# ArseneAmoya/image-retrieval-wavelet

Hardware: AMD Instinct MI355X
Metric: query images/sec + mAP@5000, MIRFLICKR-25k 64-bit hash, 1/2/4/8 MI355X (higher is better)
Workload: dtype f32; 1 GPU; c1: MIRFLICKR-25k shape, retrieval-only: per GPU per step 2048 query images 3x224x224 u8 -> SWT db2 L3 -> band-attention head (Nq=4, E=384; DINOv2 backbone out of scope, CLS features synthetic) -> 64-bit hash -> Hamming top-5000 vs 25,000 codes -> mAP@5000; queries_per_gpu=2048, db_codes=25000, nbits=64, k=5000, wavelet=db2, level=3, arithmetic=fp32 SWT and head (fp32 MFMA), 64-bit popcount ranking, AP in fp32/fp64, streams=1, clock_steps=40, backend=none, parallelism=single GPU

## Files before the change

### image-retrieval-wavelet_amd/csrc/ap_walk.hpp

```cpp
#pragma once
#include "common.hpp"

namespace wv {

constexpr int kApRounds = 32;

template <int TPQ>
__host__ __device__ constexpr int ap_scratch_dwords() { return kApRounds * (TPQ / 64) + 2 * (TPQ / 64) + 2; }

struct ApState {
    uint32_t running = 0;
    double acc = 0.0;
};

template <int TPQ>
__device__ __forceinline__ void ap_accum(uint32_t relbits, const uint32_t *cnt, int Rc, int r_base, int t, ApState &st)
{
    constexpr int NW = TPQ / 64, CH = 8;
    const int wv = t >> 6;
    for (int r0 = 0; r0 < Rc; r0 += CH) {
        uint32_t c[CH][NW];
#pragma unroll
        for (int u = 0; u < CH; ++u)
#pragma unroll
            for (int w2 = 0; w2 < NW; ++w2) c[u][w2] = cnt[min(r0 + u, Rc - 1) * NW + w2];
#pragma unroll
        for (int u = 0; u < CH; ++u) {
            const int r = r0 + u;
            if (r < Rc) {
                uint32_t before = st.running, tot = 0;
#pragma unroll
                for (int w2 = 0; w2 < NW; ++w2) {
                    before += w2 < wv ? c[u][w2] : 0u;
                    tot += c[u][w2];
                }
                const bool rel = (relbits >> r) & 1u;
                const uint64_t m = __ballot(rel);
                if (rel) {
                    const uint32_t j = before + (uint32_t)mbcnt(m) + 1;
                    st.acc += (double)((float)j / (float)((r_base + r) * TPQ + t + 1));
                }
                st.running += tot;
            }
        }
    }
}

template <int TPQ, typename SYNC>
__device__ __forceinline__ void ap_final(const ApState &st, double *wsum, int t, float *__restrict__ ap_out,
                                         int32_t *__restrict__ nrel_out, SYNC group_barrier)
{
    constexpr int NW = TPQ / 64;
    const int lane = t & 63, wv = t >> 6;
    const double acc = wave_sum_f64(st.acc);
    if (lane == 0) wsum[wv] = acc;
    group_barrier();
    if (t == 0) {
        double s = wsum[0];
#pragma unroll
        for (int w2 = 1; w2 < NW; ++w2) s += wsum[w2];
        *ap_out = st.running ? (float)(s / (double)st.running) : 0.0f;
        if (nrel_out) *nrel_out = (int32_t)st.running;
    }
}

constexpr int kMaxCutoffs = 16;

struct ApCuts {
    int n;
    int k[kMaxCutoffs];
};

template <int TPQ>
__host__ __device__ constexpr int ap_cuts_scratch_dwords() { return ap_scratch_dwords<TPQ>() + TPQ / 64; }

template <int TPQ, typename SYNC>
__device__ __forceinline__ void ap_accum_cuts(uint32_t relbits, const uint32_t *cnt, int Rc, int r_base, int t, ApState &st,
                                              const ApCuts &cuts, int &next, double *wsum, uint32_t *wcut,
                                              float *__restrict__ ap_out, int32_t *__restrict__ nrel_out, SYNC group_barrier)
{
    constexpr int NW = TPQ / 64, CH = 8;
    const int lane = t & 63, wv = t >> 6;
    int64_t cut = next < cuts.n ? cuts.k[next] : INT64_MAX;
    for (int r0 = 0; r0 < Rc; r0 += CH) {
        uint32_t c[CH][NW];
#pragma unroll
        for (int u = 0; u < CH; ++u)
#pragma unroll
            for (int w2 = 0; w2 < NW; ++w2) c[u][w2] = cnt[min(r0 + u, Rc - 1) * NW + w2];
#pragma unroll
        for (int u = 0; u < CH; ++u) {
            const int r = r0 + u;
            if (r < Rc) {
                uint32_t before = st.running, tot = 0;
#pragma unroll
                for (int w2 = 0; w2 < NW; ++w2) {
                    before += w2 < wv ? c[u][w2] : 0u;
                    tot += c[u][w2];
                }
                const bool rel = (relbits >> r) & 1u;
                const uint64_t m = __ballot(rel);
                const int p = (r_base + r) * TPQ + t;
                double own = 0.0;
                if (rel) {
                    const uint32_t j = before + (uint32_t)mbcnt(m) + 1;
                    own = (double)((float)j / (float)(p + 1));
                }
                while (cut <= (int64_t)(r_base + r + 1) * TPQ) {
                    const bool in = rel && p < cut;
                    const uint64_t mc = __ballot(in);
                    const double acc = wave_sum_f64(in ? st.acc + own : st.acc);
                    if (lane == 0) {
                        wsum[wv] = acc;
                        wcut[wv] = (uint32_t)__popcll(mc);
                    }
                    group_barrier();
                    if (t == 0) {
                        double s = wsum[0];
                        uint32_t running = st.running + wcut[0];
#pragma unroll
                        for (int w2 = 1; w2 < NW; ++w2) {
                            s += wsum[w2];
                            running += wcut[w2];
                        }
                        ap_out[next] = running ? (float)(s / (double)running) : 0.0f;
                        if (nrel_out) nrel_out[next] = (int32_t)running;
                    }
                    group_barrier();
                    ++next;
                    cut = next < cuts.n ? cuts.k[next] : INT64_MAX;
                }
                if (rel) st.acc += own;
                st.running += tot;
            }
        }
    }
}

}
```

### image-retrieval-wavelet_amd/csrc/rank.hpp

```cpp
#pragma once
#include "common.hpp"

namespace wv {

struct ApCuts;

constexpr int kTopkThreads = 256;
constexpr int kMaxBins = 130;
constexpr int kWinBins = 32;
constexpr int kWinRows = kWinBins + 1;
constexpr size_t kRankLdsLimit = 100 * 1024;

enum class RankKernel {
    none,
    column,
    window256,
    window64,
};

enum class RankMode {
    lists,
    rows16,
    hist,
    ap,
    relbits,
    radius,
};

constexpr int64_t kImg64MaxRows = 64 * 64;
constexpr int64_t kImg256MaxRows = 256 * 128;

constexpr int rank_threads_per_query(RankKernel kern) { return kern == RankKernel::window64 ? 64 : 256; }

struct RankPlan {
    RankKernel kernel;
    int C;
    int NC;
    size_t lds;
    const char *why;
    const char *instead;
};

__host__ __device__ inline int rank2_bitmap_words(int64_t N) { return (int)((N + 31) / 32); }

inline size_t window_lds_bytes_per_query(int tpq, int k, int bm_words = 0)
{
    size_t b = (size_t)kWinRows * (tpq / 2) * 4;
    b += ((size_t)(k + tpq) * 2 + 15) / 16 * 16;
    b += (size_t)(kMaxBins + 1 + kWinBins + 4 + 3) / 4 * 4 * 4;
    b += (size_t)bm_words * 4;
    b = (b + 15) / 16 * 16;
    const size_t hist = (size_t)(kMaxBins + 1) * 17 * 4;
    return b > hist ? b : (hist + 15) / 16 * 16;
}

constexpr int rank_radius_bitmap_words(int C) { return 8 * C + 1; }
inline size_t radius_lds_bytes(int C)
{
    const size_t b = (size_t)(kMaxBins + 1) * 16 * 4 + (size_t)2 * (kMaxBins + 1) * 4 + (size_t)rank_radius_bitmap_words(C) * 4;
    return (b + 15) / 16 * 16;
}

inline bool column_u16(int64_t n_items) { return n_items < 65536; }
inline size_t column_lds_bytes(int nbins, bool u16)
{
    const size_t h = (size_t)nbins * (u16 ? kTopkThreads / 2 : kTopkThreads);
    return (h + kMaxBins + kMaxBins + 1 + 4 + 3) / 4 * 4 * sizeof(uint32_t);
}

inline RankPlan rank_plan_column(int64_t N, int nbits)
{
    return {RankKernel::column, (int)ceil_div(N, kTopkThreads), 0, column_lds_bytes(nbits + 1, column_u16(N)), nullptr, ""};
}

inline RankKernel rank_window_kernel(int Q, int64_t N, int k)
{
    const char *force = ::wv::tune("WV_TOPK_V2");
    if (force && force[0] == '0') return RankKernel::none;
    if (N >= 65536 || 2 * (k + 128) >= 65536) return RankKernel::none;
    const bool fits256 = N <= kImg256MaxRows && window_lds_bytes_per_query(256, k) <= kRankLdsLimit;
    const bool fits64 = N <= kImg64MaxRows && 4 * window_lds_bytes_per_query(64, k) <= kRankLdsLimit;
    if (force && atoi(force) == 64 && fits64) return RankKernel::window64;
    if (force && atoi(force) == 256 && fits256) return RankKernel::window256;
    if (fits64 && Q >= 4096) return RankKernel::window64;
    return fits256 ? RankKernel::window256 : (fits64 ? RankKernel::window64 : RankKernel::none);
}

inline RankPlan rank_plan(int Q, int64_t N, int nbits, int k, RankMode mode)
{
    const bool fused = mode == RankMode::ap || mode == RankMode::relbits;
    const char *instead = mode == RankMode::ap ? "; call wv_hamming_topk + wv_map_at_k instead" : "";
    RankKernel kern = rank_window_kernel(Q, N, std::max(k, 1));
    if (kern == RankKernel::none) {
        if (mode == RankMode::lists) return rank_plan_column(N, nbits);
        return {RankKernel::none, 0, 0, 0, "are outside the windowed kernel (rows <= 32768, 16-bit row numbers: 2 (k + 128) < 65536)",
                instead};
    }
    if (fused && kern == RankKernel::window64 && k > 32 * 64) kern = RankKernel::window256;
    if (mode == RankMode::radius) kern = RankKernel::window256;
    RankPlan p{kern, 0, 0, 0, nullptr, ""};
    const int tpq = rank_threads_per_query(kern);
    p.C = (int)ceil_div(N, tpq);
    p.NC = p.C <= 16 ? 4 : (p.C <= 32 ? 8 : (p.C <= 64 ? 16 : (p.C <= 100 ? 25 : 32)));
    p.lds = window_lds_bytes_per_query(tpq, k, fused ? rank2_bitmap_words(N) : 0) * (kTopkThreads / tpq);
    if (mode == RankMode::radius) p.lds = radius_lds_bytes(p.C);
    if (fused && p.lds > kRankLdsLimit)
        return {RankKernel::none, 0, 0, 0, "do not fit the fused kernel's LDS (list + relevance bitmap)", instead};
    return p;
}

inline int rank_refuse(const char *what, const RankPlan &p, int64_t N, int k)
{
    WV_FAIL(WV_ENOTSUP, "%s: %lld rows / k=%d %s%s", what, (long long)N, k, p.why, p.instead);
}

inline size_t rank_image_bytes(RankKernel kern, int64_t N, int words)
{
    if (kern == RankKernel::column) return (size_t)ceil_div(N, kTopkThreads) * kTopkThreads * words * sizeof(uint64_t);
    const int tpq = rank_threads_per_query(kern);
    const int64_t C = ceil_div(N, tpq), rows = words == 1 ? (C + 1) / 2 : C;
    return (size_t)rows * tpq * 16;
}

struct BlobLayout {
    size_t column, window256, window64, total;
};
inline BlobLayout blob_layout(int64_t N, int words)
{
    BlobLayout L;
    L.column = L.window256 = L.window64 = L.total = (size_t)align_up((int64_t)dist_prepared_bytes(N, words), 256);
    if (words > 2) return L;
    L.window256 = L.column + (size_t)align_up((int64_t)rank_image_bytes(RankKernel::column, N, words), 256);
    L.window64 = L.window256 + (N <= kImg256MaxRows ? (size_t)align_up((int64_t)rank_image_bytes(RankKernel::window256, N, words), 256) : 0);
    L.total = L.window64 + (N <= kImg64MaxRows ? rank_image_bytes(RankKernel::window64, N, words) : 0);
    return L;
}
inline const void *blob_image(const void *prepared, int64_t N, int words, RankKernel kern)
{
    const BlobLayout L = blob_layout(N, words);
    return (const char *)prepared + (kern == RankKernel::column ? L.column : (kern == RankKernel::window256 ? L.window256 : L.window64));
}

int rank2_prepare(const uint64_t *db, void *img, int64_t N, int words, RankKernel kern, hipStream_t st);
size_t rank2_labels_bytes(int64_t N, int lwords);
int rank2_labels_prepare(const uint64_t *dblab, void *cls, int64_t N, int lwords, hipStream_t st);

struct Rank2Ap {
    const uint32_t *cls;
    const uint64_t *qlab;
    int lwords;
    float *ap;
    int32_t *nrel;
    uint64_t *relbits;
    int64_t relbits_ld;
    int64_t cum_ld;
};

int rank2_launch(const RankPlan &plan, const uint64_t *q, const void *img, int32_t *idx, uint16_t *rows16, uint8_t *dist,
                 uint32_t *cum, int Q, int64_t N, int nbits, int k, int64_t idx_offset, hipStream_t st,
                 const Rank2Ap *apx = nullptr, const ApCuts *cuts = nullptr);

int rank2_radius_launch(const RankPlan &plan, const uint64_t *q, const void *img, const Rank2Ap &apx, uint32_t *cum, uint32_t *cumrel,
                        int Q, int64_t N, int nbits, hipStream_t st);

}
```

### image-retrieval-wavelet_amd/csrc/rank2.hip

```cpp
#include "rank.hpp"
#include "ap_walk.hpp"

namespace wv {

#ifdef WV_RANK2_STAMPS
__device__ unsigned long long g_rank2_stamps[8];
#define R2_STAMP(i) do { __builtin_amdgcn_sched_barrier(0); const unsigned long long now_ = __builtin_amdgcn_s_memtime(); \
    __builtin_amdgcn_s_waitcnt(0xC07F); if (t == 0) atomicAdd(&g_rank2_stamps[i], now_ - stamp_); stamp_ = __builtin_amdgcn_s_memtime(); \
    __builtin_amdgcn_sched_barrier(0); } while (0)
#define R2_STAMP_INIT unsigned long long stamp_ = __builtin_amdgcn_s_memtime()
#else
#define R2_STAMP(i) do { } while (0)
#define R2_STAMP_INIT do { } while (0)
#endif

template <int WORDS>
struct QCode {
    uint64_t w[WORDS];
};

template <int TPQ>
__device__ __forceinline__ void group_sync()
{
    if constexpr (TPQ == 64) {
        __builtin_amdgcn_fence(__ATOMIC_ACQ_REL, "wavefront");
        __builtin_amdgcn_wave_barrier();
    } else {
        __syncthreads();
    }
}

__device__ __forceinline__ uint32_t wave_min_u32(uint32_t v)
{
#pragma unroll
    for (int d = 32; d > 0; d >>= 1) v = min(v, (uint32_t)__shfl_xor((int)v, d, 64));
    return v;
}

struct Rank2Lds {
    uint32_t *table;
    uint16_t *stage;
    uint32_t *gbase;
    uint32_t *tot;
    uint32_t *misc;
};

template <int WORDS, int TPQ, int NC>
__device__ __forceinline__ void rank2_distances(const uint4 *__restrict__ img, const QCode<WORDS> &qc, int64_t N, int C,
                                                int t, uint32_t (&dc)[NC], uint32_t &dmin)
{
    constexpr int UNR = WORDS == 1 ? 16 : 8;
    constexpr int LPB = WORDS == 1 ? UNR / 2 : UNR;
    const int first = t * C;
    const int nvalid = min(C, max(0, (int)N - first));
    const int rows = WORDS == 1 ? (C + 1) / 2 : C;
    const uint32_t toff = (uint32_t)t * 16u;
    dmin = 255;
#pragma unroll
    for (int i = 0; i < NC; ++i) dc[i] = 0xffffffffu;
#pragma unroll
    for (int bi = 0; bi < (NC * 4 + UNR - 1) / UNR; ++bi) {
        if (bi * UNR < C) {
            uint4 raw[LPB];
#pragma unroll
            for (int u = 0; u < LPB; ++u)
                raw[u] = *reinterpret_cast<const uint4 *>(reinterpret_cast<const char *>(img) +
                                                          (size_t)min(bi * LPB + u, rows - 1) * (TPQ * 16) + toff);
#pragma unroll
            for (int u4 = 0; u4 < UNR / 4; ++u4) {
                if (bi * (UNR / 4) + u4 >= NC) continue;
                uint32_t word = 0;
#pragma unroll
                for (int j = 0; j < 4; ++j) {
                    const int u = 4 * u4 + j;
                    uint32_t d;
                    if constexpr (WORDS == 1) {
                        const uint4 v = raw[u >> 1];
                        const uint32_t lo32 = (u & 1) ? v.z : v.x, hi32 = (u & 1) ? v.w : v.y;
                        d = (uint32_t)__popc(lo32 ^ (uint32_t)qc.w[0]) + (uint32_t)__popc(hi32 ^ (uint32_t)(qc.w[0] >> 32));
                    } else {
                        const uint4 v = raw[u];
                        d = (uint32_t)__popc(v.x ^ (uint32_t)qc.w[0]) + (uint32_t)__popc(v.y ^ (uint32_t)(qc.w[0] >> 32)) +
                            (uint32_t)__popc(v.z ^ (uint32_t)qc.w[1]) + (uint32_t)__popc(v.w ^ (uint32_t)(qc.w[1] >> 32));
                    }
                    dmin = min(dmin, d);
                    word |= d << (8 * j);
                }
                dc[bi * (UNR / 4) + u4] = word;
            }
        }
    }
#pragma unroll
    for (int i = 0; i < NC; ++i) {
        const int keep = min(4, max(0, C - 4 * i));
        dc[i] |= keep >= 4 ? 0u : (0xffffffffu << (8 * keep));
    }
    if (nvalid < C) {
#pragma unroll
        for (int i = 0; i < NC; ++i) {
            const int keep = min(4, max(0, nvalid - 4 * i));
            dc[i] |= keep >= 4 ? 0u : (0xffffffffu << (8 * keep));
        }
    }
}

template <int TPQ, int NC>
__device__ __forceinline__ void rank2_hist_only(const uint32_t (&dc)[NC], int64_t N, int C, int nbins,
                                                uint32_t *__restrict__ cum_out, uint8_t *lds_raw, int t)
{
    uint32_t *table = reinterpret_cast<uint32_t *>(lds_raw);
    uint32_t *tot = table + (kMaxBins + 1) * 16;
    for (int i = t; i < (nbins + 1) * 16; i += TPQ) table[i] = 0;
    group_sync<TPQ>();
    const uint32_t c = (uint32_t)(t & 31);
    const uint32_t cell_addr = (c >> 1) * 4u, cell_inc = 1u << (16 * (c & 1));
    char *tbl = reinterpret_cast<char *>(table);
#pragma unroll
    for (int bw = 0; bw < NC; bw += 2) {
        if (bw * 4 < C) {
#pragma unroll
            for (int j = 0; j < 8; ++j) {
                if (bw + (j >> 2) < NC) {
                    const uint32_t d = (dc[bw + (j >> 2)] >> (8 * (j & 3))) & 0xffu;
                    const uint32_t b = min(d, (uint32_t)nbins);
                    __hip_atomic_fetch_add(reinterpret_cast<uint32_t *>(tbl + b * 64 + cell_addr), cell_inc,
                                           __ATOMIC_RELAXED, __HIP_MEMORY_SCOPE_WORKGROUP);
                }
            }
            __builtin_amdgcn_sched_barrier(0);
        }
    }
    group_sync<TPQ>();
    for (int b = t; b < nbins; b += TPQ) {
        const uint4 *row = reinterpret_cast<const uint4 *>(table + b * 16);
        uint32_t s = 0;
#pragma unroll
        for (int i = 0; i < 4; ++i) {
            const uint4 v = row[i];
            s += (v.x & 0xffffu) + (v.x >> 16) + (v.y & 0xffffu) + (v.y >> 16) + (v.z & 0xffffu) + (v.z >> 16) +
                 (v.w & 0xffffu) + (v.w >> 16);
        }
        tot[b] = s;
    }
    group_sync<TPQ>();
    if (t < 64) {
        const int b0 = 3 * t;
        const uint32_t t0 = b0 < nbins ? tot[b0] : 0u, t1 = b0 + 1 < nbins ? tot[b0 + 1] : 0u, t2 = b0 + 2 < nbins ? tot[b0 + 2] : 0u;
        const uint32_t incl = wave_incl_scan_u32(t0 + t1 + t2), excl = incl - (t0 + t1 + t2);
        if (b0 <= nbins) cum_out[b0] = excl;
        if (b0 + 1 <= nbins) cum_out[b0 + 1] = excl + t0;
        if (b0 + 2 <= nbins) cum_out[b0 + 2] = excl + t0 + t1;
    }
    group_sync<TPQ>();
    (void)N;
}

template <int TPQ>
__device__ __forceinline__ void rank2_relevance_bitmap(const uint32_t *__restrict__ cls, uint64_t ql, uint64_t ql_hi, int nw, int t,
                                                       uint32_t *bitmap)
{
    constexpr int WPT = 4;
    uint32_t acc[WPT] = {0u, 0u, 0u, 0u};
    int wi[WPT];
#pragma unroll
    for (int i = 0; i < WPT; ++i) wi[i] = min(t + i * TPQ, nw - 1);
    uint64_t m = ql;
    int cbase = 0;
    if (!m) { m = ql_hi; ql_hi = 0; cbase = 64; }
    while (m) {
        const int c0 = cbase + __builtin_ctzll(m);
        m &= m - 1;
        const int c1 = m ? cbase + __builtin_ctzll(m) : c0;
        m &= m - 1;
        const int c2 = m ? cbase + __builtin_ctzll(m) : c0;
        m &= m - 1;
        const int c3 = m ? cbase + __builtin_ctzll(m) : c0;
        m &= m - 1;
        uint32_t v[4][WPT];
#pragma unroll
        for (int i = 0; i < WPT; ++i) {
            v[0][i] = cls[(size_t)c0 * nw + wi[i]];
            v[1][i] = cls[(size_t)c1 * nw + wi[i]];
            v[2][i] = cls[(size_t)c2 * nw + wi[i]];
            v[3][i] = cls[(size_t)c3 * nw + wi[i]];
        }
#pragma unroll
        for (int i = 0; i < WPT; ++i) acc[i] |= (v[0][i] | v[1][i]) | (v[2][i] | v[3][i]);
        if (!m && ql_hi) { m = ql_hi; ql_hi = 0; cbase = 64; }
    }
#pragma unroll
    for (int i = 0; i < WPT; ++i)
        if (t + i * TPQ < nw) bitmap[t + i * TPQ] = acc[i];
    for (int w = t + WPT * TPQ; w < nw; w += TPQ) bitmap[w] = 0;
}

template <int TPQ>
__device__ __forceinline__ void rank2_ap(const uint16_t *stage, const uint32_t *bitmap, uint32_t *scratch, int k, int t,
                                         float *__restrict__ ap_out, int32_t *__restrict__ nrel_out,
                                         uint64_t *__restrict__ relbits_out)
{
    constexpr int NW = TPQ / 64;
    const int lane = t & 63, wv = t >> 6;
    const int R = (k + TPQ - 1) / TPQ;
    uint32_t *cnt = scratch;
    double *wsum = reinterpret_cast<double *>(scratch + kApRounds * NW + (kApRounds * NW & 1));
    constexpr int CH = 8;
    ApState st;
    for (int c0 = 0; c0 < R; c0 += kApRounds) {
        const int Rc = min(kApRounds, R - c0);
        uint32_t relbits = 0;
        for (int r0 = c0; r0 < c0 + Rc; r0 += CH) {
            uint32_t it[CH], wd[CH];
#pragma unroll
            for (int u = 0; u < CH; ++u) it[u] = stage[min((r0 + u) * TPQ + t, k - 1)];
#pragma unroll
            for (int u = 0; u < CH; ++u) wd[u] = bitmap[it[u] >> 5];
#pragma unroll
            for (int u = 0; u < CH; ++u) {
                const int r = r0 + u;
                const bool rel = r < c0 + Rc && r * TPQ + t < k && ((wd[u] >> (it[u] & 31)) & 1u);
                relbits |= (rel ? 1u : 0u) << ((r - c0) & 31);
                const uint64_t m = __ballot(rel);
                if (lane == 0 && r < c0 + Rc) {
                    if (!relbits_out) cnt[(r - c0) * NW + wv] = (uint32_t)__popcll(m);
                    else if ((r * NW + wv) * 64 < k) relbits_out[r * NW + wv] = m;
                }
            }
        }
        if (relbits_out) continue;
        group_sync<TPQ>();
        ap_accum<TPQ>(relbits, cnt, Rc, c0, t, st);
        group_sync<TPQ>();
    }
    if (relbits_out) return;
    ap_final<TPQ>(st, wsum, t, ap_out, nrel_out, [] { group_sync<TPQ>(); });
}
template <int TPQ>
__device__ __forceinline__ void rank2_ap_cuts(const uint16_t *stage, const uint32_t *bitmap, uint32_t *scratch, int k, int t,
                                              float *__restrict__ ap_out, int32_t *__restrict__ nrel_out, const ApCuts &cuts)
{
    constexpr int NW = TPQ / 64, CH = 8;
    const int lane = t & 63, wv = t >> 6;
    const int R = (k + TPQ - 1) / TPQ;
    uint32_t *cnt = scratch;
    double *wsum = reinterpret_cast<double *>(scratch + kApRounds * NW + (kApRounds * NW & 1));
    uint32_t *wcut = reinterpret_cast<uint32_t *>(wsum + NW);
    ApState st;
    int next = 0;
    for (int c0 = 0; c0 < R; c0 += kApRounds) {
        const int Rc = min(kApRounds, R - c0);
        uint32_t relbits = 0;
        for (int r0 = c0; r0 < c0 + Rc; r0 += CH) {
            uint32_t it[CH], wd[CH];
#pragma unroll
            for (int u = 0; u < CH; ++u) it[u] = stage[min((r0 + u) * TPQ + t, k - 1)];
#pragma unroll
            for (int u = 0; u < CH; ++u) wd[u] = bitmap[it[u] >> 5];
#pragma unroll
            for (int u = 0; u < CH; ++u) {
                const int r = r0 + u;
                const bool rel = r < c0 + Rc && r * TPQ + t < k && ((wd[u] >> (it[u] & 31)) & 1u);
                relbits |= (rel ? 1u : 0u) << ((r - c0) & 31);
                const uint64_t m = __ballot(rel);
                if (lane == 0 && r < c0 + Rc) cnt[(r - c0) * NW + wv] = (uint32_t)__popcll(m);
            }
        }
        group_sync<TPQ>();
        ap_accum_cuts<TPQ>(relbits, cnt, Rc, c0, t, st, cuts, next, wsum, wcut, ap_out, nrel_out, [] { group_sync<TPQ>(); });
        group_sync<TPQ>();
    }
}

template <int TPQ>
__device__ __forceinline__ Rank2Lds rank2_lds(uint8_t *lds_raw, int k)
{
    Rank2Lds L;
    L.table = reinterpret_cast<uint32_t *>(lds_raw);
    uint8_t *p = lds_raw + (size_t)kWinRows * TPQ * 2;
    L.stage = reinterpret_cast<uint16_t *>(p);
    p += ((size_t)(k + TPQ) * 2 + 15) / 16 * 16;
    L.gbase = reinterpret_cast<uint32_t *>(p);
    L.tot = L.gbase + kMaxBins + 1;
    L.misc = L.tot + kWinBins;
    return L;
}

template <int TPQ>
__device__ __forceinline__ void rank2_zero_table(uint8_t *lds_raw, int t)
{
    uint4 *t4 = reinterpret_cast<uint4 *>(lds_raw);
    constexpr int n4 = kWinRows * TPQ * 2 / 16;
    for (int i = t; i < n4; i += TPQ) t4[i] = make_uint4(0, 0, 0, 0);
}

template <int TPQ>
__device__ __forceinline__ void rank2_copy_list(uint8_t *lds_raw, int k, int64_t idx_offset, int32_t *__restrict__ idx_out,
                                                uint16_t *__restrict__ rows16_out, int t)
{
    const Rank2Lds L = rank2_lds<TPQ>(lds_raw, k);
    if (rows16_out) {
        if ((k & 7) == 0 && (reinterpret_cast<uintptr_t>(rows16_out) & 15) == 0) {
            const uint4 *s4 = reinterpret_cast<const uint4 *>(L.stage);
            uint4 *o4 = reinterpret_cast<uint4 *>(rows16_out);
            for (int i = t; i < k / 8; i += TPQ) o4[i] = s4[i];
        } else {
            for (int i = t; i < k; i += TPQ) rows16_out[i] = L.stage[i];
        }
    } else if (idx_out) {
        const bool vec = (k & 3) == 0 && (reinterpret_cast<uintptr_t>(idx_out) & 15) == 0;
        const int32_t off = (int32_t)idx_offset;
        if (vec) {
            const uint2 *s2 = reinterpret_cast<const uint2 *>(L.stage);
            int4 *o4 = reinterpret_cast<int4 *>(idx_out);
            for (int i = t; i < k / 4; i += TPQ) {
                const uint2 v = s2[i];
                o4[i] = make_int4((int32_t)(v.x & 0xffffu) + off, (int32_t)(v.x >> 16) + off,
                                  (int32_t)(v.y & 0xffffu) + off, (int32_t)(v.y >> 16) + off);
            }
        } else {
            for (int i = t; i < k; i += TPQ) idx_out[i] = (int32_t)L.stage[i] + off;
        }
    }
}

template <int TPQ>
__device__ __forceinline__ void rank2_dist_row(const Rank2Lds &L, int nbins, int k, uint8_t *__restrict__ dist_out, int t)
{
    {
        const uintptr_t a0 = reinterpret_cast<uintptr_t>(dist_out);
        for (int p0 = t * 16; p0 < k; p0 += TPQ * 16) {
            int a = 0, z = nbins;
            while (z - a > 1) {
                const int mid = (a + z) >> 1;
                if (L.gbase[mid] <= (uint32_t)p0) a = mid;
                else z = mid;
            }
            int bin = a;
            uint32_t next = L.gbase[bin + 1];
            uint32_t w4[4];
#pragma unroll
            for (int j4 = 0; j4 < 4; ++j4) {
                uint32_t word = 0;
#pragma unroll
                for (int j = 0; j < 4; ++j) {
                    const uint32_t pp = (uint32_t)(p0 + 4 * j4 + j);
                    while (pp >= next && bin + 1 < nbins) { ++bin; next = L.gbase[bin + 1]; }
                    word |= (uint32_t)bin << (8 * j);
                }
                w4[j4] = word;
            }
            if (((a0 + p0) & 15) == 0 && p0 + 16 <= k) {
                *reinterpret_cast<uint4 *>(dist_out + p0) = make_uint4(w4[0], w4[1], w4[2], w4[3]);
            } else if (((a0 + p0) & 3) == 0) {
#pragma unroll
                for (int j4 = 0; j4 < 4; ++j4) {
                    if (p0 + 4 * j4 + 4 <= k) {
                        *reinterpret_cast<uint32_t *>(dist_out + p0 + 4 * j4) = w4[j4];
                    } else {
                        for (int j = 0; j < 4; ++j)
                            if (p0 + 4 * j4 + j < k) dist_out[p0 + 4 * j4 + j] = (uint8_t)(w4[j4] >> (8 * j));
                    }
                }
            } else {
                for (int j = 0; j < 16; ++j)
                    if (p0 + j < k) dist_out[p0 + j] = (uint8_t)(w4[j >> 2] >> (8 * (j & 3)));
            }
        }
    }
}

template <int TPQ, int NC, int AP = 0>
__device__ __forceinline__ void rank2_rank(const uint32_t (&dc)[NC], uint32_t dmin, int64_t N, int C, int nbins, int k,
                                           uint32_t *__restrict__ cum_out, uint8_t *__restrict__ dist_out, uint8_t *lds_raw, int t,
                                           const uint32_t *__restrict__ cls = nullptr, uint64_t qlabel = 0, uint64_t qlabel_hi = 0,
                                           float *__restrict__ ap_out = nullptr, int32_t *__restrict__ nrel_out = nullptr,
                                           uint64_t *__restrict__ relbits_out = nullptr, const ApCuts *cuts = nullptr)
{
    constexpr int ROWB = TPQ * 2;
    const Rank2Lds L = rank2_lds<TPQ>(lds_raw, k);
    uint32_t *bitmap = L.misc + 4;
    R2_STAMP_INIT;
    if constexpr (AP) rank2_relevance_bitmap<TPQ>(cls, qlabel, qlabel_hi, rank2_bitmap_words(N), t, bitmap);
    R2_STAMP(6);
    const int lane = t & 63, wv = __builtin_amdgcn_readfirstlane(t >> 6);
    constexpr int NW = TPQ / 64;
    const int first = t * C;
    dmin = wave_min_u32(dmin);
    if constexpr (NW > 1) {
        if (lane == 0) L.misc[wv] = dmin;
        __syncthreads();
        dmin = min(min(L.misc[0], L.misc[1]), min(L.misc[2], L.misc[3]));
    }
    for (int b = t; b <= nbins; b += TPQ) L.gbase[b] = b <= (int)dmin ? 0u : 0xffffffffu;
    int lo = min((int)dmin, nbins - 1);
    uint32_t placed = 0;
    const uint32_t cell_addr = (uint32_t)((t >> 6) * 32 + (t & 31)) * 4u;
    const uint32_t cell_shift = 16u * ((t >> 5) & 1);
    const uint32_t cell_inc = 2u << cell_shift;
    char *tbl = reinterpret_cast<char *>(L.table);
    char *stage_b = reinterpret_cast<char *>(L.stage);
    const uint32_t trash = 2u * (uint32_t)(k + t);
    const uint32_t k2 = 2u * (uint32_t)k;

    R2_STAMP(0);
    for (;;) {
        const bool place = placed < (uint32_t)k;
        char *row0 = tbl + cell_addr;
#pragma unroll
        for (int bw = 0; bw < NC; bw += 2) {
            if (bw * 4 < C) {
#pragma unroll
                for (int j = 0; j < 8; ++j) {
                    if (bw + (j >> 2) < NC) {
                        const uint32_t d = (dc[bw + (j >> 2)] >> (8 * (j & 3))) & 0xffu;
                        const uint32_t b = min(d - (uint32_t)lo, (uint32_t)kWinBins);
                        __hip_atomic_fetch_add(reinterpret_cast<uint32_t *>(row0 + b * ROWB), cell_inc,
                                               __ATOMIC_RELAXED, __HIP_MEMORY_SCOPE_WORKGROUP);
                    }
                }
            }
        }
        group_sync<TPQ>();
        R2_STAMP(1);
        uint32_t win_total, bin_base;
        if constexpr (TPQ == 64) {
            for (int b = 0; b < kWinBins; ++b) {
                uint32_t s2 = (L.table[b * (TPQ / 2) + (lane & 31)] >> cell_shift) & 0xffffu;
                s2 = wave_sum_u32(s2) >> 1;
                if (lane == 0) L.tot[b] = s2;
            }
            group_sync<TPQ>();
            const uint32_t my_tot = lane < kWinBins ? L.tot[lane] : 0u;
            const uint32_t incl = wave_incl_scan_u32(my_tot);
            bin_base = placed + incl - my_tot;
            win_total = (uint32_t)__builtin_amdgcn_readlane((int)incl, 63);
            if (lane < kWinBins && lo + lane + 1 <= nbins) L.gbase[lo + lane + 1] = placed + incl;
            if (place) {
                for (int b = 0; b < kWinBins; ++b) {
                    const uint32_t base_b = (uint32_t)__builtin_amdgcn_readlane((int)bin_base, b);
                    const uint32_t c = (L.table[b * (TPQ / 2) + (lane & 31)] >> cell_shift) & 0xffffu;
                    const uint32_t excl = wave_incl_scan_u32(c) - c + 2u * base_b;
                    reinterpret_cast<uint16_t *>(L.table + b * (TPQ / 2))[2 * (lane & 31) + (lane >> 5)] = (uint16_t)min(excl, k2);
                }
            }
        } else {
            for (int b = wv; b < kWinBins; b += NW) {
                const uint2 v = *reinterpret_cast<const uint2 *>(L.table + b * (TPQ / 2) + 2 * lane);
                uint32_t s2 = (v.x & 0xffffu) + (v.x >> 16) + (v.y & 0xffffu) + (v.y >> 16);
                s2 = wave_sum_u32(s2) >> 1;
                if (lane == 0) L.tot[b] = s2;
            }
            group_sync<TPQ>();
            const uint32_t my_tot = lane < kWinBins ? L.tot[lane] : 0u;
            const uint32_t incl = wave_incl_scan_u32(my_tot);
            bin_base = placed + incl - my_tot;
            win_total = (uint32_t)__builtin_amdgcn_readlane((int)incl, 63);
            if (wv == 0 && lane < kWinBins && lo + lane + 1 <= nbins) L.gbase[lo + lane + 1] = placed + incl;
            if (place) {
                const int t0 = 4 * lane, d0 = (t0 >> 6) * 32 + (t0 & 31), sh = 16 * ((t0 >> 5) & 1);
                for (int b = wv; b < kWinBins; b += NW) {
                    const uint32_t base_b = (uint32_t)__builtin_amdgcn_readlane((int)bin_base, b);
                    const uint4 v = *reinterpret_cast<const uint4 *>(L.table + b * (TPQ / 2) + d0);
                    const uint32_t c0 = (v.x >> sh) & 0xffffu, c1 = (v.y >> sh) & 0xffffu, c2 = (v.z >> sh) & 0xffffu,
                                   c3 = (v.w >> sh) & 0xffffu;
                    const uint32_t s4 = c0 + c1 + c2 + c3;
                    const uint32_t e0 = wave_incl_scan_u32(s4) - s4 + 2u * base_b;
                    const uint32_t e1 = e0 + c0, e2 = e1 + c1, e3 = e2 + c2;
                    uint16_t *h = reinterpret_cast<uint16_t *>(L.table + b * (TPQ / 2) + d0) + (sh >> 4);
                    h[0] = (uint16_t)min(e0, k2); h[2] = (uint16_t)min(e1, k2); h[4] = (uint16_t)min(e2, k2); h[6] = (uint16_t)min(e3, k2);
                }
            }
        }
        if (place) {
            if (wv == NW - 1) {
                const uint32_t kk = k2 * 0x10001u;
                for (int i = lane; i < TPQ / 2; i += 64) L.table[kWinBins * (TPQ / 2) + i] = kk;
            }
            group_sync<TPQ>();
            R2_STAMP(2);
#pragma unroll
            for (int bw = 0; bw < NC; bw += 4) {
                if (bw * 4 < C) {
                    uint32_t old[16];
#pragma unroll
                    for (int j = 0; j < 16; ++j) {
                        old[j] = 0;
                        if (bw + (j >> 2) < NC) {
                            const uint32_t d = (dc[bw + (j >> 2)] >> (8 * (j & 3))) & 0xffu;
                            const uint32_t b = min(d - (uint32_t)lo, (uint32_t)kWinBins);
                            old[j] = __hip_atomic_fetch_add(reinterpret_cast<uint32_t *>(row0 + b * ROWB), cell_inc,
                                                            __ATOMIC_RELAXED, __HIP_MEMORY_SCOPE_WORKGROUP);
                        }
                    }
#pragma unroll
                    for (int j = 0; j < 16; ++j) {
                        if (bw + (j >> 2) < NC) {
                            const uint32_t pos2 = (old[j] >> cell_shift) & 0xffffu;
                            *reinterpret_cast<uint16_t *>(stage_b + min(pos2, trash)) =
                                (uint16_t)(first + bw * 4 + j);
                        }
                    }
                    __builtin_amdgcn_sched_barrier(0);
                }
            }
        }
        R2_STAMP(3);
        placed += win_total;
        lo += kWinBins;
        if (lo >= nbins || (placed >= (uint32_t)k && !cum_out)) break;
        group_sync<TPQ>();
        rank2_zero_table<TPQ>(lds_raw, t);
        group_sync<TPQ>();
    }
    group_sync<TPQ>();
    if (cum_out)
        for (int b = t; b <= nbins; b += TPQ) cum_out[b] = min(L.gbase[b], (uint32_t)N);
    if (dist_out) rank2_dist_row<TPQ>(L, nbins, k, dist_out, t);
    R2_STAMP(4);
    if constexpr (AP) {
        if constexpr (AP == 2) rank2_ap_cuts<TPQ>(L.stage, bitmap, L.table, k, t, ap_out, nrel_out, *cuts);
        else rank2_ap<TPQ>(L.stage, bitmap, L.table, k, t, ap_out, nrel_out, relbits_out);
        R2_STAMP(7);
        group_sync<TPQ>();
    }
}

template <int WORDS>
__global__ __launch_bounds__(256) void k_rank2_image(const uint64_t *__restrict__ db, uint4 *__restrict__ img, int64_t N,
                                                     int C, int tpq)
{
    const int rows = WORDS == 1 ? (C + 1) / 2 : C;
    const int64_t total = (int64_t)rows * tpq;
    for (int64_t i = (int64_t)blockIdx.x * blockDim.x + threadIdx.x; i < total; i += (int64_t)gridDim.x * blockDim.x) {
        const int64_t r = i / tpq;
        const int t = (int)(i - r * tpq);
        uint64_t a = 0, b = 0;
        if constexpr (WORDS == 1) {
            const int64_t i0 = 2 * r, i1 = 2 * r + 1, it0 = (int64_t)t * C + i0, it1 = (int64_t)t * C + i1;
            if (i0 < C && it0 < N) a = db[it0];
            if (i1 < C && it1 < N) b = db[it1];
        } else {
            const int64_t it = (int64_t)t * C + r;
            if (it < N) { a = db[it * 2]; b = db[it * 2 + 1]; }
        }
        img[i] = make_uint4((uint32_t)a, (uint32_t)(a >> 32), (uint32_t)b, (uint32_t)(b >> 32));
    }
}

__global__ __launch_bounds__(256) void k_rank2_label_matrix(const uint64_t *__restrict__ dblab, uint32_t *__restrict__ cls, int64_t N,
                                                            int nw, int lwords)
{
    const int ncls = 64 * lwords;
    const int64_t i = (int64_t)blockIdx.x * 256 + threadIdx.x;
    if (i >= (int64_t)nw * ncls) return;
    const int c = (int)(i % ncls);
    const int64_t w = i / ncls;
    uint32_t word = 0;
    for (int j = 0; j < 32; ++j) {
        const int64_t r = w * 32 + j;
        if (r < N) word |= (uint32_t)((dblab[r * lwords + (c >> 6)] >> (c & 63)) & 1ull) << j;
    }
    cls[(size_t)c * nw + w] = word;
}

size_t rank2_labels_bytes(int64_t N, int lwords) { return (size_t)64 * lwords * rank2_bitmap_words(N) * sizeof(uint32_t); }

int rank2_labels_prepare(const uint64_t *dblab, void *cls, int64_t N, int lwords, hipStream_t st)
{
    const int nw = rank2_bitmap_words(N);
    hipLaunchKernelGGL(k_rank2_label_matrix, dim3((unsigned)ceil_div((int64_t)nw * 64 * lwords, 256)), dim3(256), 0, st, dblab,
                       (uint32_t *)cls, N, nw, lwords);
    WV_CHECK_LAUNCH("k_rank2_label_matrix");
    return WV_OK;
}

constexpr int rank2_min_waves(int nc) { return nc <= 8 ? 7 : (nc <= 16 ? 6 : (nc <= 25 ? 5 : (nc <= 50 ? 4 : 3))); }

template <int WORDS, int TPQ, int NC, bool AP>
__global__ __launch_bounds__(256, rank2_min_waves(NC)) void k_rank_window(const uint64_t *__restrict__ q, const uint4 *__restrict__ img,
                                                     int32_t *__restrict__ idx, uint16_t *__restrict__ rows16,
                                                     uint8_t *__restrict__ dist, int Q, int64_t N, int C, int nbins, int k,
                                                     int64_t idx_offset, uint32_t *__restrict__ cum, int lds_per_group, Rank2Ap apx)
{
    extern __shared__ uint4 lds4[];
    constexpr int GPW = 256 / TPQ;
    const int g = threadIdx.x / TPQ, t = threadIdx.x % TPQ;
    const int qi = blockIdx.x * GPW + g;
    if (qi >= Q) return;
    uint8_t *lds = reinterpret_cast<uint8_t *>(lds4) + (size_t)g * lds_per_group;
    QCode<WORDS> qc;
#pragma unroll
    for (int w = 0; w < WORDS; ++w) {
        const uint64_t v = q[(int64_t)qi * WORDS + w];
        qc.w[w] = ((uint64_t)(uint32_t)__builtin_amdgcn_readfirstlane((int)(uint32_t)(v >> 32)) << 32) |
                  (uint32_t)__builtin_amdgcn_readfirstlane((int)(uint32_t)v);
    }
    if (k != 0) rank2_zero_table<TPQ>(lds, t);
    uint32_t dc[NC], dmin;
    rank2_distances<WORDS, TPQ, NC>(img, qc, N, C, t, dc, dmin);
#pragma unroll
    for (int once = 0; once < 1; ++once) {
        if (k == 0) {
            rank2_hist_only<TPQ, NC>(dc, N, C, nbins, cum + (int64_t)qi * (nbins + 1), lds, t);
            continue;
// ... 266 lines not shown
```

Baseline: 1.602 million query images/s.

## Scatter relevance bytes instead of item ids in fused AP rank kernel

In the fused rank+AP kernel, the placement pass now writes a one-byte relevance flag per ranked position, looked up from the bitmap at scatter time, instead of a 16-bit item id. These bytes are packed into a 64-bit relevance string, and the AP walk reads whole words with popcount prefix scans and readlane, replacing the per-round ballot/count table and its group barriers. This is meant to remove the indirect stage-to-bitmap gathers and the per-chunk LDS synchronisation, and it shrinks the LDS footprint per query. The cost is a bit-packing pass, plus changed LDS layout and trash-slot arithmetic that must stay correct.

```diff
diff --git a/image-retrieval-wavelet_amd/csrc/ap_walk.hpp b/image-retrieval-wavelet_amd/csrc/ap_walk.hpp
--- a/image-retrieval-wavelet_amd/csrc/ap_walk.hpp
+++ b/image-retrieval-wavelet_amd/csrc/ap_walk.hpp
@@ -64,6 +64,69 @@
     }
 }
 
+template <int TPQ>
+struct ApWords {
+    static constexpr int NW = TPQ / 64, WPL = (kApRounds * NW + 63) / 64;
+    uint64_t w[WPL];
+    uint32_t ex[WPL];
+    uint32_t total;
+};
+
+template <int TPQ>
+__device__ __forceinline__ ApWords<TPQ> ap_words_load(const uint64_t *str, int nwords, int Rc, int r_base, int lane)
+{
+    constexpr int NW = ApWords<TPQ>::NW, WPL = ApWords<TPQ>::WPL;
+    ApWords<TPQ> a;
+    uint32_t carry = 0;
+#pragma unroll
+    for (int i = 0; i < WPL; ++i) {
+        const int wl = i * 64 + lane, wi = r_base * NW + wl;
+        a.w[i] = (wl < Rc * NW && wi < nwords) ? str[wi] : 0ull;
+        const uint32_t c = (uint32_t)__popcll(a.w[i]), incl = wave_incl_scan_u32(c);
+        a.ex[i] = carry + incl - c;
+        carry += (uint32_t)__builtin_amdgcn_readlane((int)incl, 63);
+    }
+    a.total = carry;
+    return a;
+}
+
+template <int TPQ>
+__device__ __forceinline__ void ap_words_round(const ApWords<TPQ> &a, int r, int wv, uint64_t &m, uint32_t &before,
+                                               uint32_t &before_round)
+{
+    constexpr int NW = ApWords<TPQ>::NW, WPL = ApWords<TPQ>::WPL;
+    const int wl = r * NW + wv, sel = wl >> 6, ln = wl & 63;
+    uint64_t ws = a.w[0];
+    uint32_t es = a.ex[0];
+#pragma unroll
+    for (int i = 1; i < WPL; ++i)
+        if (sel == i) {
+            ws = a.w[i];
+            es = a.ex[i];
+        }
+    m = ((uint64_t)(uint32_t)__builtin_amdgcn_readlane((int)(uint32_t)(ws >> 32), ln) << 32) |
+        (uint32_t)__builtin_amdgcn_readlane((int)(uint32_t)ws, ln);
+    before = (uint32_t)__builtin_amdgcn_readlane((int)es, ln);
+    before_round = (uint32_t)__builtin_amdgcn_readlane((int)es, ln - wv);
+}
+
+template <int TPQ>
+__device__ __forceinline__ void ap_accum_words(const uint64_t *str, int nwords, int Rc, int r_base, int t, ApState &st)
+{
+    const int lane = t & 63, wv = __builtin_amdgcn_readfirstlane(t >> 6);
+    const ApWords<TPQ> a = ap_words_load<TPQ>(str, nwords, Rc, r_base, lane);
+    for (int r = 0; r < Rc; ++r) {
+        uint64_t m;
+        uint32_t before, before_round;
+        ap_words_round<TPQ>(a, r, wv, m, before, before_round);
+        if ((m >> lane) & 1ull) {
+            const uint32_t j = st.running + before + (uint32_t)mbcnt(m) + 1;
+            st.acc += (double)((float)j / (float)((r_base + r) * TPQ + t + 1));
+        }
+    }
+    st.running += a.total;
+}
+
 constexpr int kMaxCutoffs = 16;
 
 struct ApCuts {
@@ -75,12 +138,52 @@
 __host__ __device__ constexpr int ap_cuts_scratch_dwords() { return ap_scratch_dwords<TPQ>() + TPQ / 64; }
 
 template <int TPQ, typename SYNC>
+__device__ __forceinline__ void ap_cut_round(bool rel, uint64_t m, uint32_t before, uint32_t running, int round, int t, ApState &st,
+                                             const ApCuts &cuts, int &next, int64_t &cut, double *wsum, uint32_t *wcut,
+                                             float *__restrict__ ap_out, int32_t *__restrict__ nrel_out, SYNC group_barrier)
+{
+    constexpr int NW = TPQ / 64;
+    const int lane = t & 63, wv = t >> 6;
+    const int p = round * TPQ + t;
+    double own = 0.0;
+    if (rel) {
+        const uint32_t j = before + (uint32_t)mbcnt(m) + 1;
+        own = (double)((float)j / (float)(p + 1));
+    }
+    while (cut <= (int64_t)(round + 1) * TPQ) {
+        const bool in = rel && p < cut;
+        const uint64_t mc = __ballot(in);
+        const double acc = wave_sum_f64(in ? st.acc + own : st.acc);
+        if (lane == 0) {
+            wsum[wv] = acc;
+            wcut[wv] = (uint32_t)__popcll(mc);
+        }
+        group_barrier();
+        if (t == 0) {
+            double s = wsum[0];
+            uint32_t hits = running + wcut[0];
+#pragma unroll
+            for (int w2 = 1; w2 < NW; ++w2) {
+                s += wsum[w2];
+                hits += wcut[w2];
+            }
+            ap_out[next] = hits ? (float)(s / (double)hits) : 0.0f;
+            if (nrel_out) nrel_out[next] = (int32_t)hits;
+        }
+        group_barrier();
+        ++next;
+        cut = next < cuts.n ? cuts.k[next] : INT64_MAX;
+    }
+    if (rel) st.acc += own;
+}
+
+template <int TPQ, typename SYNC>
 __device__ __forceinline__ void ap_accum_cuts(uint32_t relbits, const uint32_t *cnt, int Rc, int r_base, int t, ApState &st,
                                               const ApCuts &cuts, int &next, double *wsum, uint32_t *wcut,
                                               float *__restrict__ ap_out, int32_t *__restrict__ nrel_out, SYNC group_barrier)
 {
     constexpr int NW = TPQ / 64, CH = 8;
-    const int lane = t & 63, wv = t >> 6;
+    const int wv = t >> 6;
     int64_t cut = next < cuts.n ? cuts.k[next] : INT64_MAX;
     for (int r0 = 0; r0 < Rc; r0 += CH) {
         uint32_t c[CH][NW];
@@ -100,41 +203,30 @@
                 }
                 const bool rel = (relbits >> r) & 1u;
                 const uint64_t m = __ballot(rel);
-                const int p = (r_base + r) * TPQ + t;
-                double own = 0.0;
-                if (rel) {
-                    const uint32_t j = before + (uint32_t)mbcnt(m) + 1;
-                    own = (double)((float)j / (float)(p + 1));
-                }
-                while (cut <= (int64_t)(r_base + r + 1) * TPQ) {
-                    const bool in = rel && p < cut;
-                    const uint64_t mc = __ballot(in);
-                    const double acc = wave_sum_f64(in ? st.acc + own : st.acc);
-                    if (lane == 0) {
-                        wsum[wv] = acc;
-                        wcut[wv] = (uint32_t)__popcll(mc);
-                    }
-                    group_barrier();
-                    if (t == 0) {
-                        double s = wsum[0];
-                        uint32_t running = st.running + wcut[0];
-#pragma unroll
-                        for (int w2 = 1; w2 < NW; ++w2) {
-                            s += wsum[w2];
-                            running += wcut[w2];
-                        }
-                        ap_out[next] = running ? (float)(s / (double)running) : 0.0f;
-                        if (nrel_out) nrel_out[next] = (int32_t)running;
-                    }
-                    group_barrier();
-                    ++next;
-                    cut = next < cuts.n ? cuts.k[next] : INT64_MAX;
-                }
-                if (rel) st.acc += own;
+                ap_cut_round<TPQ>(rel, m, before, st.running, r_base + r, t, st, cuts, next, cut, wsum, wcut, ap_out, nrel_out,
+                                  group_barrier);
                 st.running += tot;
             }
         }
     }
 }
 
-}
+template <int TPQ, typename SYNC>
+__device__ __forceinline__ void ap_accum_cuts_words(const uint64_t *str, int nwords, int Rc, int r_base, int t, ApState &st,
+                                                    const ApCuts &cuts, int &next, double *wsum, uint32_t *wcut,
+                                                    float *__restrict__ ap_out, int32_t *__restrict__ nrel_out, SYNC group_barrier)
+{
+    const int lane = t & 63, wv = __builtin_amdgcn_readfirstlane(t >> 6);
+    const ApWords<TPQ> a = ap_words_load<TPQ>(str, nwords, Rc, r_base, lane);
+    int64_t cut = next < cuts.n ? cuts.k[next] : INT64_MAX;
+    for (int r = 0; r < Rc; ++r) {
+        uint64_t m;
+        uint32_t before, before_round;
+        ap_words_round<TPQ>(a, r, wv, m, before, before_round);
+        ap_cut_round<TPQ>((m >> lane) & 1ull, m, st.running + before, st.running + before_round, r_base + r, t, st, cuts, next, cut,
+                          wsum, wcut, ap_out, nrel_out, group_barrier);
+    }
+    st.running += a.total;
+}
+
+}
diff --git a/image-retrieval-wavelet_amd/csrc/rank.hpp b/image-retrieval-wavelet_amd/csrc/rank.hpp
--- a/image-retrieval-wavelet_amd/csrc/rank.hpp
+++ b/image-retrieval-wavelet_amd/csrc/rank.hpp
@@ -43,10 +43,11 @@
 
 __host__ __device__ inline int rank2_bitmap_words(int64_t N) { return (int)((N + 31) / 32); }
 
-inline size_t window_lds_bytes_per_query(int tpq, int k, int bm_words = 0)
+inline size_t window_lds_bytes_per_query(int tpq, int k, int bm_words = 0, bool fused = false)
 {
     size_t b = (size_t)kWinRows * (tpq / 2) * 4;
-    b += ((size_t)(k + tpq) * 2 + 15) / 16 * 16;
+    if (fused) b += ((size_t)(k + 63) / 64 * 8 + (size_t)k + (size_t)tpq * 4 + 8 + 15) / 16 * 16;
+    else b += ((size_t)(k + tpq) * 2 + 15) / 16 * 16;
     b += (size_t)(kMaxBins + 1 + kWinBins + 4 + 3) / 4 * 4 * 4;
     b += (size_t)bm_words * 4;
     b = (b + 15) / 16 * 16;
@@ -102,10 +103,10 @@
     const int tpq = rank_threads_per_query(kern);
     p.C = (int)ceil_div(N, tpq);
     p.NC = p.C <= 16 ? 4 : (p.C <= 32 ? 8 : (p.C <= 64 ? 16 : (p.C <= 100 ? 25 : 32)));
-    p.lds = window_lds_bytes_per_query(tpq, k, fused ? rank2_bitmap_words(N) : 0) * (kTopkThreads / tpq);
+    p.lds = window_lds_bytes_per_query(tpq, k, fused ? rank2_bitmap_words(N) + 1 : 0, fused) * (kTopkThreads / tpq);
     if (mode == RankMode::radius) p.lds = radius_lds_bytes(p.C);
     if (fused && p.lds > kRankLdsLimit)
-        return {RankKernel::none, 0, 0, 0, "do not fit the fused kernel's LDS (list + relevance bitmap)", instead};
+        return {RankKernel::none, 0, 0, 0, "do not fit the fused kernel's LDS (position relevance + relevance bitmap)", instead};
     return p;
 }
 
diff --git a/image-retrieval-wavelet_amd/csrc/rank2.hip b/image-retrieval-wavelet_amd/csrc/rank2.hip
--- a/image-retrieval-wavelet_amd/csrc/rank2.hip
+++ b/image-retrieval-wavelet_amd/csrc/rank2.hip
@@ -40,6 +40,8 @@
 struct Rank2Lds {
     uint32_t *table;
     uint16_t *stage;
+    uint64_t *str;
+    uint8_t *rel8;
     uint32_t *gbase;
     uint32_t *tot;
     uint32_t *misc;
@@ -195,90 +197,46 @@
 }
 
 template <int TPQ>
-__device__ __forceinline__ void rank2_ap(const uint16_t *stage, const uint32_t *bitmap, uint32_t *scratch, int k, int t,
-                                         float *__restrict__ ap_out, int32_t *__restrict__ nrel_out,
-                                         uint64_t *__restrict__ relbits_out)
+__device__ __forceinline__ void rank2_ap(const uint64_t *str, uint32_t *scratch, int k, int t, float *__restrict__ ap_out,
+                                         int32_t *__restrict__ nrel_out, uint64_t *__restrict__ relbits_out)
+{
+    const int nwords = (k + 63) / 64;
+    if (relbits_out) {
+        for (int i = t; i < nwords; i += TPQ) relbits_out[i] = str[i];
+        return;
+    }
+    const int R = (k + TPQ - 1) / TPQ;
+    ApState st;
+    for (int c0 = 0; c0 < R; c0 += kApRounds)
+        ap_accum_words<TPQ>(str, nwords, min(kApRounds, R - c0), c0, t, st);
+    ap_final<TPQ>(st, reinterpret_cast<double *>(scratch), t, ap_out, nrel_out, [] { group_sync<TPQ>(); });
+}
+template <int TPQ>
+__device__ __forceinline__ void rank2_ap_cuts(const uint64_t *str, uint32_t *scratch, int k, int t, float *__restrict__ ap_out,
+                                              int32_t *__restrict__ nrel_out, const ApCuts &cuts)
 {
     constexpr int NW = TPQ / 64;
-    const int lane = t & 63, wv = t >> 6;
-    const int R = (k + TPQ - 1) / TPQ;
-    uint32_t *cnt = scratch;
-    double *wsum = reinterpret_cast<double *>(scratch + kApRounds * NW + (kApRounds * NW & 1));
-    constexpr int CH = 8;
-    ApState st;
-    for (int c0 = 0; c0 < R; c0 += kApRounds) {
-        const int Rc = min(kApRounds, R - c0);
-        uint32_t relbits = 0;
-        for (int r0 = c0; r0 < c0 + Rc; r0 += CH) {
-            uint32_t it[CH], wd[CH];
-#pragma unroll
-            for (int u = 0; u < CH; ++u) it[u] = stage[min((r0 + u) * TPQ + t, k - 1)];
-#pragma unroll
-            for (int u = 0; u < CH; ++u) wd[u] = bitmap[it[u] >> 5];
-#pragma unroll
-            for (int u = 0; u < CH; ++u) {
-                const int r = r0 + u;
-                const bool rel = r < c0 + Rc && r * TPQ + t < k && ((wd[u] >> (it[u] & 31)) & 1u);
-                relbits |= (rel ? 1u : 0u) << ((r - c0) & 31);
-                const uint64_t m = __ballot(rel);
-                if (lane == 0 && r < c0 + Rc) {
-                    if (!relbits_out) cnt[(r - c0) * NW + wv] = (uint32_t)__popcll(m);
-                    else if ((r * NW + wv) * 64 < k) relbits_out[r * NW + wv] = m;
-                }
-            }
-        }
-        if (relbits_out) continue;
-        group_sync<TPQ>();
-        ap_accum<TPQ>(relbits, cnt, Rc, c0, t, st);
-        group_sync<TPQ>();
-    }
-    if (relbits_out) return;
-    ap_final<TPQ>(st, wsum, t, ap_out, nrel_out, [] { group_sync<TPQ>(); });
-}
-template <int TPQ>
-__device__ __forceinline__ void rank2_ap_cuts(const uint16_t *stage, const uint32_t *bitmap, uint32_t *scratch, int k, int t,
-                                              float *__restrict__ ap_out, int32_t *__restrict__ nrel_out, const ApCuts &cuts)
-{
-    constexpr int NW = TPQ / 64, CH = 8;
-    const int lane = t & 63, wv = t >> 6;
-    const int R = (k + TPQ - 1) / TPQ;
-    uint32_t *cnt = scratch;
-    double *wsum = reinterpret_cast<double *>(scratch + kApRounds * NW + (kApRounds * NW & 1));
+    const int nwords = (k + 63) / 64, R = (k + TPQ - 1) / TPQ;
+    double *wsum = reinterpret_cast<double *>(scratch);
     uint32_t *wcut = reinterpret_cast<uint32_t *>(wsum + NW);
     ApState st;
     int next = 0;
-    for (int c0 = 0; c0 < R; c0 += kApRounds) {
-        const int Rc = min(kApRounds, R - c0);
-        uint32_t relbits = 0;
-        for (int r0 = c0; r0 < c0 + Rc; r0 += CH) {
-            uint32_t it[CH], wd[CH];
-#pragma unroll
-            for (int u = 0; u < CH; ++u) it[u] = stage[min((r0 + u) * TPQ + t, k - 1)];
-#pragma unroll
-            for (int u = 0; u < CH; ++u) wd[u] = bitmap[it[u] >> 5];
-#pragma unroll
-            for (int u = 0; u < CH; ++u) {
-                const int r = r0 + u;
-                const bool rel = r < c0 + Rc && r * TPQ + t < k && ((wd[u] >> (it[u] & 31)) & 1u);
-                relbits |= (rel ? 1u : 0u) << ((r - c0) & 31);
-                const uint64_t m = __ballot(rel);
-                if (lane == 0 && r < c0 + Rc) cnt[(r - c0) * NW + wv] = (uint32_t)__popcll(m);
-            }
-        }
-        group_sync<TPQ>();
-        ap_accum_cuts<TPQ>(relbits, cnt, Rc, c0, t, st, cuts, next, wsum, wcut, ap_out, nrel_out, [] { group_sync<TPQ>(); });
-        group_sync<TPQ>();
-    }
-}
-
-template <int TPQ>
+    for (int c0 = 0; c0 < R; c0 += kApRounds)
+        ap_accum_cuts_words<TPQ>(str, nwords, min(kApRounds, R - c0), c0, t, st, cuts, next, wsum, wcut, ap_out, nrel_out,
+                                 [] { group_sync<TPQ>(); });
+}
+
+template <int TPQ, bool FUSED = false>
 __device__ __forceinline__ Rank2Lds rank2_lds(uint8_t *lds_raw, int k)
 {
     Rank2Lds L;
     L.table = reinterpret_cast<uint32_t *>(lds_raw);
     uint8_t *p = lds_raw + (size_t)kWinRows * TPQ * 2;
     L.stage = reinterpret_cast<uint16_t *>(p);
-    p += ((size_t)(k + TPQ) * 2 + 15) / 16 * 16;
+    L.str = reinterpret_cast<uint64_t *>(p);
+    L.rel8 = p + (size_t)(k + 63) / 64 * 8;
+    if constexpr (FUSED) p += ((size_t)(k + 63) / 64 * 8 + (size_t)k + (size_t)TPQ * 4 + 8 + 15) / 16 * 16;
+    else p += ((size_t)(k + TPQ) * 2 + 15) / 16 * 16;
     L.gbase = reinterpret_cast<uint32_t *>(p);
     L.tot = L.gbase + kMaxBins + 1;
     L.misc = L.tot + kWinBins;
@@ -291,6 +249,20 @@
     uint4 *t4 = reinterpret_cast<uint4 *>(lds_raw);
     constexpr int n4 = kWinRows * TPQ * 2 / 16;
     for (int i = t; i < n4; i += TPQ) t4[i] = make_uint4(0, 0, 0, 0);
+}
+
+template <int TPQ>
+__device__ __forceinline__ void rank2_pack_string(const Rank2Lds &L, int k, int t)
+{
+    const uint64_t *r64 = reinterpret_cast<const uint64_t *>(L.rel8);
+    uint8_t *s8 = reinterpret_cast<uint8_t *>(L.str);
+    const int n8 = (k + 7) / 8;
+    for (int i = t; i < (k + 63) / 64 * 8; i += TPQ) {
+        uint64_t x = i < n8 ? r64[i] : 0ull;
+        if (8 * i + 8 > k) x &= (1ull << (8 * max(k - 8 * i, 0))) - 1;
+        s8[i] = (uint8_t)(((x & 0x0101010101010101ull) * 0x0102040810204080ull) >> 56);
+    }
+    group_sync<TPQ>();
 }
 
 template <int TPQ>
@@ -377,7 +349,7 @@
                                            uint64_t *__restrict__ relbits_out = nullptr, const ApCuts *cuts = nullptr)
 {
     constexpr int ROWB = TPQ * 2;
-    const Rank2Lds L = rank2_lds<TPQ>(lds_raw, k);
+    const Rank2Lds L = rank2_lds<TPQ, AP != 0>(lds_raw, k);
     uint32_t *bitmap = L.misc + 4;
     R2_STAMP_INIT;
     if constexpr (AP) rank2_relevance_bitmap<TPQ>(cls, qlabel, qlabel_hi, rank2_bitmap_words(N), t, bitmap);
@@ -394,13 +366,15 @@
     for (int b = t; b <= nbins; b += TPQ) L.gbase[b] = b <= (int)dmin ? 0u : 0xffffffffu;
     int lo = min((int)dmin, nbins - 1);
     uint32_t placed = 0;
+    constexpr uint32_t UNIT = AP ? 1u : 2u;
     const uint32_t cell_addr = (uint32_t)((t >> 6) * 32 + (t & 31)) * 4u;
     const uint32_t cell_shift = 16u * ((t >> 5) & 1);
-    const uint32_t cell_inc = 2u << cell_shift;
+    const uint32_t cell_inc = UNIT << cell_shift;
     char *tbl = reinterpret_cast<char *>(L.table);
     char *stage_b = reinterpret_cast<char *>(L.stage);
-    const uint32_t trash = 2u * (uint32_t)(k + t);
-    const uint32_t k2 = 2u * (uint32_t)k;
+    const uint32_t trash = AP ? (uint32_t)(k + 4 * t) : 2u * (uint32_t)(k + t);
+    const uint32_t k2 = UNIT * (uint32_t)k;
+    char *rel8_b = reinterpret_cast<char *>(L.rel8);
 
     R2_STAMP(0);
     for (;;) {
@@ -426,7 +400,7 @@
         if constexpr (TPQ == 64) {
             for (int b = 0; b < kWinBins; ++b) {
                 uint32_t s2 = (L.table[b * (TPQ / 2) + (lane & 31)] >> cell_shift) & 0xffffu;
-                s2 = wave_sum_u32(s2) >> 1;
+                s2 = wave_sum_u32(s2) / UNIT;
                 if (lane == 0) L.tot[b] = s2;
             }
             group_sync<TPQ>();
@@ -439,7 +413,7 @@
                 for (int b = 0; b < kWinBins; ++b) {
                     const uint32_t base_b = (uint32_t)__builtin_amdgcn_readlane((int)bin_base, b);
                     const uint32_t c = (L.table[b * (TPQ / 2) + (lane & 31)] >> cell_shift) & 0xffffu;
-                    const uint32_t excl = wave_incl_scan_u32(c) - c + 2u * base_b;
+                    const uint32_t excl = wave_incl_scan_u32(c) - c + UNIT * base_b;
                     reinterpret_cast<uint16_t *>(L.table + b * (TPQ / 2))[2 * (lane & 31) + (lane >> 5)] = (uint16_t)min(excl, k2);
                 }
             }
@@ -447,7 +421,7 @@
             for (int b = wv; b < kWinBins; b += NW) {
                 const uint2 v = *reinterpret_cast<const uint2 *>(L.table + b * (TPQ / 2) + 2 * lane);
                 uint32_t s2 = (v.x & 0xffffu) + (v.x >> 16) + (v.y & 0xffffu) + (v.y >> 16);
-                s2 = wave_sum_u32(s2) >> 1;
+                s2 = wave_sum_u32(s2) / UNIT;
                 if (lane == 0) L.tot[b] = s2;
             }
             group_sync<TPQ>();
@@ -464,7 +438,7 @@
                     const uint32_t c0 = (v.x >> sh) & 0xffffu, c1 = (v.y >> sh) & 0xffffu, c2 = (v.z >> sh) & 0xffffu,
                                    c3 = (v.w >> sh) & 0xffffu;
                     const uint32_t s4 = c0 + c1 + c2 + c3;
-                    const uint32_t e0 = wave_incl_scan_u32(s4) - s4 + 2u * base_b;
+                    const uint32_t e0 = wave_incl_scan_u32(s4) - s4 + UNIT * base_b;
                     const uint32_t e1 = e0 + c0, e2 = e1 + c1, e3 = e2 + c2;
                     uint16_t *h = reinterpret_cast<uint16_t *>(L.table + b * (TPQ / 2) + d0) + (sh >> 4);
                     h[0] = (uint16_t)min(e0, k2); h[2] = (uint16_t)min(e1, k2); h[4] = (uint16_t)min(e2, k2); h[6] = (uint16_t)min(e3, k2);
@@ -481,7 +455,11 @@
 #pragma unroll
             for (int bw = 0; bw < NC; bw += 4) {
                 if (bw * 4 < C) {
-                    uint32_t old[16];
+                    uint32_t old[16], rel16 = 0;
+                    if constexpr (AP != 0) {
+                        const int p = first + bw * 4, w = min(p >> 5, rank2_bitmap_words(N) - 1);
+                        rel16 = (uint32_t)((((uint64_t)bitmap[w + 1] << 32) | bitmap[w]) >> (p & 31));
+                    }
 #pragma unroll
                     for (int j = 0; j < 16; ++j) {
                         old[j] = 0;
@@ -496,8 +474,12 @@
                     for (int j = 0; j < 16; ++j) {
                         if (bw + (j >> 2) < NC) {
                             const uint32_t pos2 = (old[j] >> cell_shift) & 0xffffu;
-                            *reinterpret_cast<uint16_t *>(stage_b + min(pos2, trash)) =
-                                (uint16_t)(first + bw * 4 + j);
+                            if constexpr (AP != 0) {
+                                *reinterpret_cast<uint8_t *>(rel8_b + min(pos2, trash)) = (uint8_t)((rel16 >> j) & 1u);
+                            } else {
+                                *reinterpret_cast<uint16_t *>(stage_b + min(pos2, trash)) =
+                                    (uint16_t)(first + bw * 4 + j);
+                            }
                         }
                     }
                     __builtin_amdgcn_sched_barrier(0);
@@ -518,8 +500,9 @@
     if (dist_out) rank2_dist_row<TPQ>(L, nbins, k, dist_out, t);
     R2_STAMP(4);
     if constexpr (AP) {
-        if constexpr (AP == 2) rank2_ap_cuts<TPQ>(L.stage, bitmap, L.table, k, t, ap_out, nrel_out, *cuts);
-        else rank2_ap<TPQ>(L.stage, bitmap, L.table, k, t, ap_out, nrel_out, relbits_out);
+        rank2_pack_string<TPQ>(L, k, t);
+        if constexpr (AP == 2) rank2_ap_cuts<TPQ>(L.str, L.table, k, t, ap_out, nrel_out, *cuts);
+        else rank2_ap<TPQ>(L.str, L.table, k, t, ap_out, nrel_out, relbits_out);
         R2_STAMP(7);
         group_sync<TPQ>();
     }
```

Measured after the change: 1.599 million query images/s. About the same (-0.2%).
